# ini/multigrid

Measured on AMD Instinct MI355X. Metric: agent-steps/sec, higher is better.
Workload: dtype u8

## Files before the change

### multigrid_amd/csrc/mgx_fused.h

```cpp
#pragma once
#if !defined(__HIPCC_RTC__)
#include <hip/hip_runtime.h>
#include <limits.h>
#include <stdint.h>
#else
namespace __hip_internal {}
using namespace __hip_internal;
typedef unsigned long uintptr_t;
#ifndef offsetof
#define offsetof(t, m) __builtin_offsetof(t, m)
#endif
#ifndef INT_MAX
#define INT_MAX 2147483647
#endif
#ifndef INT64_MAX
#define INT64_MAX 9223372036854775807LL
#endif
#endif

#include "mgx_rules.h"
#include "mgx_layout_gen.h"

namespace mgx_fused {

// ... 463 lines not shown
        for (int n = 0; n < NH; ++n) {
            uint32_t t, addr;
            asm("v_pk_max_i16 %0, %1, %2" : "=v"(t) : "v"(lc.pk[0]), "v"(r[n].lo));
            asm("v_pk_min_i16 %0, %1, %2" : "=v"(t) : "v"(t), "v"(r[n].hi));
            asm("v_dot2_i32_i16 %0, %1, %2, %3" : "=v"(addr) : "v"(t), "v"(r[n].steps), "v"(r[n].origin));
            MGX_CHECK_LDS_ADDR(4, addr, C8 ? 1 : 2);
            raw[h0 + n] = gather_read<C8>(addr);
        }
        if (h0 + NH < N) __builtin_amdgcn_sched_barrier(0);
    }
#pragma unroll
    for (int p = 0; p < NP; ++p) {
        constexpr int kLast = N - 3 * (NP - 1);
        const int ns = p == NP - 1 ? kLast : 3;
        const int sub16 = ns == 3 ? lc.sub16 : min(lc.sub16, (ns - 1) * (int)sizeof(ViewRec));
        const ViewRec r = *reinterpret_cast<const ViewRec *>(reinterpret_cast<const uint8_t *>(rec + S0 + 3 * p) + sub16);
        uint32_t t, addr;
        asm("v_pk_max_i16 %0, %1, %2" : "=v"(t) : "v"(lc.pk[1]), "v"(r.lo));
        asm("v_pk_min_i16 %0, %1, %2" : "=v"(t) : "v"(t), "v"(r.hi));
        asm("v_dot2_i32_i16 %0, %1, %2, %3" : "=v"(addr) : "v"(t), "v"(r.steps), "v"(r.origin));
        if (lc.act[1]) MGX_CHECK_LDS_ADDR(4, addr, C8 ? 1 : 2);
        rawR[p] = gather_read<C8>(addr);
    }
    [[maybe_unused]] uint32_t dec[C8 ? N : 1], decR[C8 ? NP : 1];
    if constexpr (C8) {
#pragma unroll
        for (int n = 0; n < N; ++n) {
            MGX_CHECK_LDS_ADDR(9, lut_mid + (raw[n] << 2), 4);
            dec[n] = lut_decode(raw[n], lut_mid);
        }
#pragma unroll
        for (int p = 0; p < NP; ++p) {
            if (lc.act[1]) MGX_CHECK_LDS_ADDR(9, lut_mid + (rawR[p] << 2), 4);
            decR[p] = lut_decode(rawR[p], lut_mid);
        }
    }
    uint64_t pend = 0;
#pragma unroll
    for (int n = 0; n < N; ++n) {
        if constexpr (HALF) {
            if ((n & 1) == 0) cell[(S0 + n) >> 1][0] = raw[n] | (raw[n + 1] << 16);
        } else if constexpr (C8) {
            cell[S0 + n][0] = dec[n];
        } else {
            cell[S0 + n][0] = raw[n];
        }
        uint64_t cur;
        if (n == 0) {
            asm volatile("v_cmp_lt_i16_e64 %0, -1, %1\n\ts_nop 1" : "=s"(cur) : "v"(raw[n]));
        } else {
            asm volatile("v_cmp_lt_i16_e64 %0, -1, %3\n\tv_writelane_b32 %1, %4, %6\n\tv_writelane_b32 %2, %5, %6"
                         : "=&s"(cur), "+v"(sbLo[0]), "+v"(sbHi[0])
                         : "v"(raw[n]), "s"((uint32_t)pend), "s"((uint32_t)(pend >> 32)), "n"(S0 + n - 1));
        }
        pend = cur;
    }
    asm volatile("s_nop 1\n\tv_writelane_b32 %0, %2, %4\n\tv_writelane_b32 %1, %3, %4"
                 : "+v"(sbLo[0]), "+v"(sbHi[0]) : "s"((uint32_t)pend), "s"((uint32_t)(pend >> 32)), "n"(S0 + N - 1));
#pragma unroll
    for (int p = 0; p < NP; ++p) {
        constexpr int kLast = N - 3 * (NP - 1);
        const int ns = p == NP - 1 ? kLast : 3;
        if constexpr (C8) cell[pk3_reg<N>(S0, p)][1] = decR[p];
        else cell[pk3_reg<N>(S0, p)][1] = rawR[p];
        uint64_t cur;
        asm volatile("v_cmp_lt_i16_e64 %0, -1, %1" : "=s"(cur) : "v"(rawR[p]));
        constexpr uint32_t kWord = (1u << R) - 1u;
#pragma unroll
        for (int q = 0; q < 3; ++q) {
            if (q < ns) {
                const uint32_t part = (uint32_t)(cur >> (R * q)) & kWord;
                asm volatile("v_writelane_b32 %0, %1, %2" : "+v"(sbLo[1]) : "s"(part), "n"(S0 + 3 * p + q));
            }
        }
    }
    (void)sbHi;
}

#ifndef MGX_GROUP
#define MGX_GROUP 16
#endif
constexpr int kGroup = MGX_GROUP;

template <int V, int NW, int VPW, bool HALF, int G, bool C8 = false, int S0 = 0>
__device__ __forceinline__ void gather_all(const KernelArgs &a, const int wave, int NVc, const ViewRec *rec,
                                           const LaneConst<V, NW> &lc, uint32_t (&cell)[HALF ? VPW / 2 : VPW][NW],
                                           uint32_t (&sbLo)[NW], uint32_t (&sbHi)[NW], const uint32_t lut_mid = 0) {
    if constexpr (S0 < VPW) {
        if (S0 < NVc) {
            if constexpr (kPack3<V>) gather_group_pk3<V, NW, S0, G, VPW, HALF, C8>(a, wave, rec, lc, cell, sbLo, sbHi, lut_mid);
            else gather_group<V, NW, S0, G, VPW, HALF, C8>(a, wave, rec, lc, cell, sbLo, sbHi, lut_mid);
        }
        gather_all<V, NW, VPW, HALF, G, C8, S0 + G>(a, wave, NVc, rec, lc, cell, sbLo, sbHi, lut_mid);
    }
}

template <int V, int MODE, bool HOOKS, bool AR, bool OH = false, bool GEN = false, bool STREAM = false, bool DMA = (MGX_LDS_DMA != 0),
          int GRP = kGroup, int SHAPE = 0, bool C8 = false, bool B3 = false>
__global__ __launch_bounds__(kMaxThreads) void mgx_fused_kernel(const KernelArgs a) {
#include "mgx_fused_body.inc"
}

template <int MODE, bool AR>
__global__ __launch_bounds__(kMaxThreads) __attribute__((amdgpu_waves_per_eu(4)))
void mgx_resident_kernel(const KernelArgs a) {
    constexpr int V = 7, GRP = kGroup, SHAPE = kShapeResident4;
    constexpr bool HOOKS = false, OH = false, GEN = false, STREAM = false, DMA = false, C8 = false, B3 = false;
#include "mgx_fused_body.inc"
}

template <int V, bool OH, bool STREAM, bool DMA, bool C8 = false, bool B3 = false>
__global__ __launch_bounds__(kMaxThreads) __attribute__((amdgpu_waves_per_eu(6)))
void mgx_obs_kernel(const KernelArgs a) {
    constexpr int MODE = 0, GRP = kGroup, SHAPE = 0;
    constexpr bool HOOKS = false, AR = false, GEN = false;
#include "mgx_fused_body.inc"
}

constexpr bool has_small_groups(int V, int MODE, bool OH, bool GEN) {
    return MGX_DEBUG_KNOBS != 0 && MODE == 1 && V <= 9 && !OH && !GEN;
}

inline int match_fixed_shape(const KernelArgs &ka, bool hooks, bool persist = false) {
    if (MGX_NO_FIXED_SHAPES || ka.grp != kGroup) return 0;
    for (int k = 1; k < kNumShapes; ++k) {
        const FixedShape &f = kShapes[k];
        if (f.ns > 0) continue;
        if (persist ? !f.dma : (((ka.flags & 2) != 0) != f.dma || ((ka.flags & 1) != 0) != f.stream)) continue;
        if (ka.sp.view_size == f.V
            && ka.sp.width == f.W && ka.sp.height == f.H && ka.sp.num_agents == f.A && ka.Gw == f.Gw && hooks == f.hooks
            && ka.vpw == shape_slots(f)
            && cell_bytes_of(ka.sp) == f.cb
            && ka.wave_lds == make_carve(f.W, f.H, f.A, f.V, f.Gw, shape_slots(f), persist, f.hooks, false, kGroup, f.cb).total())
            return k;
    }
    return 0;
}

inline int match_resident_shape(const KernelArgs &ka, bool hooks) {
    if (MGX_NO_FIXED_SHAPES || ka.grp != kGroup || ka.ns < 1 || ka.rshape < 1 || ka.rshape >= kNumShapes) return 0;
    const FixedShape &f = kShapes[ka.rshape];
    if (f.ns == ka.ns && ka.sp.view_size == f.V && ka.sp.width == f.W && ka.sp.height == f.H && ka.sp.num_agents == f.A && ka.Gw == f.Gw
        && hooks == f.hooks && ka.vpw == shape_slots(f) && cell_bytes_of(ka.sp) == f.cb && ka.wave_lds == shape_carve(f, true).total())
        return ka.rshape;
    return 0;
}

#if !defined(__HIPCC_RTC__)
struct JitShape { FixedShape f; int vpw, wave_lds; hipFunction_t fn[2]; };
const JitShape *jit_shape_lookup(const KernelArgs &ka, bool hooks);
template <int V, int MODE, bool STREAM, bool C8 = true, bool OH = false>
inline int launch_compact(const KernelArgs &ka, int threads, int lds_bytes, int64_t nwg, hipStream_t stream, int *hip_err, int *occupancy) {
    constexpr bool B3 = !C8;
    if constexpr (MODE > 1 && C8 && !OH && !STREAM) {
        if (ka.grp != kGroup || ka.vpw > 32) return MGX_ERR_INVALID_ARGUMENT;
        if (ka.sp.env_kind != MGX_KIND_EMPTY) return MGX_ERR_UNSUPPORTED;
        const bool ar = ka.pool_grid != nullptr;
        void (*kern)(const KernelArgs) = ar ? mgx_fused_kernel<V, MODE, false, true, false, false, false, false, kGroup, 0, true, false>
                                            : mgx_fused_kernel<V, MODE, false, false, false, false, false, false, kGroup, 0, true, false>;
        if (lds_bytes > 64 * 1024) {
            hipError_t e = hipFuncSetAttribute(reinterpret_cast<const void *>(kern), hipFuncAttributeMaxDynamicSharedMemorySize, lds_bytes);
            if (e != hipSuccess) { *hip_err = (int)e; (void)hipGetLastError(); return MGX_ERR_LAUNCH; }
        }
        if (occupancy) {
            hipError_t e = hipOccupancyMaxActiveBlocksPerMultiprocessor(occupancy, reinterpret_cast<const void *>(kern), threads, (size_t)lds_bytes);
            if (e != hipSuccess) { *hip_err = (int)e; (void)hipGetLastError(); return MGX_ERR_LAUNCH; }
// ... 199 lines not shown
```

### multigrid_amd/csrc/mgx_fused_body.inc

```
    constexpr bool DO_STEP = MODE != 0;
    const int env_kind = HOOKS ? a.sp.env_kind : (int)MGX_KIND_EMPTY;
    constexpr bool PERSIST = MODE == 3;
    constexpr bool ROLL = MODE == 2 || PERSIST;
    constexpr int kOutAux = PERSIST ? 16 : MGX_OUT_AUX;
#define MGX_PUB_STORE_U8(base, idx, n, val)                                                                            \
    do {                                                                                                               \
        if constexpr (PERSIST) __builtin_amdgcn_raw_buffer_store_b8((uint8_t)(val), make_rsrc((base), (n)), (idx), 0, 16); \
        else MGX_STORE_SMALL((base) + (idx), (uint8_t)(val));                                                          \
    } while (0)
    constexpr int V2 = V * V;
    constexpr int NW = (V2 + 63) / 64;
    constexpr int CB = C8 ? 1 : kCellBytes;
    static_assert(!C8 || (!GEN && !DMA && (MODE < 2 ? (!OH || (MODE == 1 && !HOOKS)) : (!OH && !HOOKS))),
                  "compact cells: the plain step / gen_obs kernels, the step with one-hot output, the hook-free rollout / persistent kernels");
    static_assert(SHAPE == 0 || kShapes[SHAPE].cb == CB, "shape table entry of the other cell format");
    static_assert(!B3 || (!C8 && !OH && !GEN && !DMA && MODE < 2 && SHAPE == 0), "byte grids: the plain step / gen_obs kernels only");
    constexpr int CBG = B3 ? 3 : CB;
    constexpr bool RSHAPE = SHAPE != 0 && kShapes[SHAPE].ns > 0;
    constexpr int NS = RSHAPE ? kShapes[SHAPE].ns : 1;
    constexpr int PITCH = RSHAPE ? kShapes[SHAPE].pitch : 0;
    constexpr bool SLICED = RSHAPE && shape_sliced(kShapes[SHAPE]);
    static_assert(!RSHAPE || ((MODE == 2 || MODE == 3) && !OH && !GEN && !STREAM && !DMA && !C8 && !B3 && V <= 7), "resident shapes: rollout / persistent kernels");
    static_assert(NS <= 2, "slices: the (step, slice) sequence below is written for one or two");
    constexpr bool HALF = !DMA && (MODE == 1 || RSHAPE) && !C8;
    constexpr bool PK3 = kPack3<V>;
    constexpr int kG = GRP, kR = SLICED ? kRoundResident : GRP;
    constexpr int kG4 = kR < kG ? kR : kG;
    constexpr int VPW = (DMA && GRP < kGroup) ? GRP : ((V <= 7 && HALF) ? kSlotsSmallView : 32);
    extern __shared__ __align__(16) uint8_t lds[];

    int lane_ = threadIdx.x & 63;
#define lane lane_

    const int wave = __builtin_amdgcn_readfirstlane(threadIdx.x >> 6);
#if MGX_EARLY_ARGS
    if constexpr ((DMA || MGX_EARLY_ARGS > 1) && V <= 7) {
        const int64_t e_batch = a.batch;
        const uint8_t *e_grid = a.grid, *e_agents = a.agents, *e_aux = a.aux, *e_hord = a.hook_order;
        const uint64_t *e_rng = a.rng;
        const int32_t *e_sc = a.step_count;
        const int8_t *e_act = a.actions;
        const unsigned e_bd = blockDim.x;
        const int32_t *e_ep = (AR || GEN) ? a.episode : nullptr;
        const uint8_t *e_trunc = DO_STEP ? a.truncated : nullptr;
        const uint64_t *e_gs = GEN ? a.gen.gen_state : nullptr;
        const int32_t *e_tag = GEN ? a.gen.stage.tag : nullptr;
        asm volatile("" :: "s"(e_batch), "s"(e_grid), "s"(e_agents), "s"(e_rng), "s"(e_sc), "s"(e_act), "s"(e_hord), "s"(e_aux),
                     "s"(e_bd), "s"(e_ep), "s"(e_trunc), "s"(e_gs), "s"(e_tag));
    }
#endif
    constexpr bool FIXED = SHAPE != 0;
    constexpr bool PREFIX = FIXED ? (kShapes[SHAPE].A > 4) : (V > 7 && MODE == 1);
    constexpr bool BIGCOPY = FIXED ? (kShapes[SHAPE].W * kShapes[SHAPE].H * CB >= 4096) : (V > 7 && MODE == 1);
    const int W = FIXED ? kShapes[SHAPE].W : a.sp.width, H = FIXED ? kShapes[SHAPE].H : a.sp.height,
              A = FIXED ? kShapes[SHAPE].A : a.sp.num_agents;
    const int Gw_ = FIXED ? kShapes[SHAPE].Gw : a.Gw;
    const int vpw_ = FIXED ? shape_slots(kShapes[SHAPE]) : a.vpw;
    const int inv_A_ = FIXED ? (65536 + kShapes[SHAPE].A - 1) / (FIXED ? kShapes[SHAPE].A : 1) : a.inv_A;
    const int HWB = H * W * CB;
    const int HWG = H * W * CBG;
#define MGX_LATE_GEN(f) kernarg_at<decltype(MgxLayoutGen::f)>(offsetof(KernelArgs, gen) + offsetof(MgxLayoutGen, f))
#define MGX_LATE_STAGE(f) kernarg_at<decltype(MgxGenStage::f)>(offsetof(KernelArgs, gen) + offsetof(MgxLayoutGen, stage) + offsetof(MgxGenStage, f))
    if constexpr (GEN && MODE == 1) {
        if ((int64_t)blockIdx.x >= a.gen_first_wg) {
            const int64_t gw = ((int64_t)blockIdx.x - a.gen_first_wg) * (blockDim.x >> 6) + wave;
            const int64_t b = gw * 64 + lane;
            int32_t *const tag = MGX_LATE_STAGE(tag);
            const int32_t phase1 = MGX_LATE_STAGE(phase) + 1;
            const bool serial = MGX_LATE_STAGE(external) == 2;
            int32_t req = b >= a.batch ? 0 : serial ? tag[b * 4 + 3]
                                                    : __hip_atomic_load(tag + b * 4 + 3, __ATOMIC_ACQUIRE, __HIP_MEMORY_SCOPE_AGENT);
            if (req != 0 && req != phase1 && tag[b * 4 + 1] != a.episode[b]) { tag[b * 4 + 3] = 0; req = 0; }
            const bool go = req != 0 && req != phase1;
            const uint64_t gom = __builtin_amdgcn_ballot_w64(go);
#if MGX_SPANS
            const int64_t wid_g = a.gen_first_wg * (blockDim.x >> 6) + gw;
            const unsigned long long t_g0 = __builtin_amdgcn_s_memrealtime();
            if (gom == 0 && lane == 0 && a.span_base + wid_g < kSpanCap) {
                g_span[2 * (a.span_base + wid_g)] = t_g0;
                g_span[2 * (a.span_base + wid_g) + 1] = __builtin_amdgcn_s_memrealtime() & 0x0fffffffffffffffull;
            }
#endif
            if (gom == 0) return;
            MGX_RARE_PATH_PRIO();
            MgxLayoutGen gen;
            gen.kind = MGX_LATE_GEN(kind); gen.room_size = MGX_LATE_GEN(room_size);
            gen.start_x = MGX_LATE_GEN(start_x); gen.start_y = MGX_LATE_GEN(start_y); gen.start_dir = MGX_LATE_GEN(start_dir);
            gen.max_hallway_keys = MGX_LATE_GEN(max_hallway_keys); gen.max_keys_per_room = MGX_LATE_GEN(max_keys_per_room);
            gen.blank = MGX_LATE_GEN(blank); gen.gen_state = MGX_LATE_GEN(gen_state);
            uint8_t *const st_grid = reinterpret_cast<uint8_t *>(MGX_LATE_STAGE(grid));
            mgx_gen::copy_blank(gen, st_grid, gw * 64, HWB, gom, lane);
            __builtin_amdgcn_fence(__ATOMIC_RELEASE, "wavefront");
            __builtin_amdgcn_s_waitcnt(0x0F70);
            wave_sync();
            if (go) {
                const int32_t ep_s = tag[b * 4 + 1], sc_s = tag[b * 4 + 2];
                uint64_t *const words = MGX_LATE_STAGE(words) + b * 12;
                const uint64_t *gs = gen.gen_state + b * 6, *rg = a.rng + b * 4;
                mgx_gen::NpGen lay, npr;
                for (int k = 0; k < 4; ++k) lay.s[k] = gs[k];
                lay.buf = gs[4]; npr.buf = gs[5];
                uint64_t s0 = words[10], s1 = words[11];
                const uint64_t i0 = rg[2], i1 = rg[3];
                const uint64_t jA[4] = {kJump.w[A][0], kJump.w[A][1], kJump.w[A][2], kJump.w[A][3]};
                if (A > 1 && a.sp.max_steps > sc_s) pcg64_advance(s0, s1, i0, i1, jA, (uint32_t)(a.sp.max_steps - sc_s));
                npr.s[0] = s0; npr.s[1] = s1; npr.s[2] = i0; npr.s[3] = i1;
                uint8_t *apos = lds + wave * a.wave_lds + lane * (2 * A);
                const uint4 naux = mgx_gen::generate_episode(gen, W, H, A, lay, npr, apos, st_grid + b * HWB,
// ... 781 lines not shown
        if (ovl >= 0) {
            MGX_CHECK_LDS_PTR(3, mytile + ovl, CB);
            store_cell_raw(CB, mytile + ovl, agent_cell_raw(CB, cur_row));
        }
    } else {
        const int off = (lane < NVc) ? overlay_offset(cf, rows + env_of_lane * A, agent_of_lane) : -1;
        wave_sync();
        if (off >= 0) store_cell_raw(CB, tile + env_of_lane * TSB + off, agent_cell_raw(CB, cur_row));
    }
    wave_sync();

    MGX_MARK("P1d");
    const uint32_t tile_addr = (uint32_t)(wave * wave_lds_ + cv.tile(sl_s) + tile_skew);
    uint32_t my_carry = 0;
    uint8_t *const p_dir = MGX_LATE(dir);
    uint8_t *const p_agents = DO_STEP ? MGX_LATE(agents) : nullptr;
    double *const p_reward = DO_STEP ? MGX_LATE(reward) : nullptr;
    uint8_t *const p_term = DO_STEP ? MGX_LATE(terminated) : nullptr;
    if (lane < NVc) {
        const int e = env_of_lane;
        const uint64_t row = cur_row;
        const ViewGeom g = view_geom<V>(W, H, row_x(row), row_y(row), row_dir(row), CB, PITCH);
        const ViewClamp vc = view_clamp<V>(g, W, H, row_x(row), row_y(row));
        ViewRec r;
        r.origin = vc.valid ? (int32_t)tile_addr + e * TSB + g.origin : (int32_t)wall_addr;
        r.steps = vc.valid ? vc.steps : 0u; r.lo = vc.valid ? vc.lo : 0u; r.hi = vc.valid ? vc.hi : 0u;
        my_carry = row_carry(row) & kCellShown;
        rec[lane] = r;
        if (DO_STEP) {
            const u32x2 rowv = {(uint32_t)row, (uint32_t)(row >> 32)};
            if (!ROLL) __builtin_amdgcn_raw_buffer_store_b64(rowv, make_rsrc(p_agents + v0 * 8, NVc * 8), lane * 8, 0,MGX_OUT_AUX);
            const uint64_t rbits = __builtin_bit_cast(uint64_t, my_rew);
            const u32x2 rewv = {(uint32_t)rbits, (uint32_t)(rbits >> 32)};
            __builtin_amdgcn_raw_buffer_store_b64(rewv, make_rsrc(p_reward + tv0, NVc * 8), lane * 8, 0, kOutAux);
            const bool forced = env_kind == MGX_KIND_LOCKEDHALLWAY && reinterpret_cast<const uint8_t *>(auxl + e)[15];
            __builtin_amdgcn_raw_buffer_store_b8((uint8_t)(row_term(row) | forced),
                                                 make_rsrc(p_term + tv0, NVc), lane, 0, kOutAux);
        }
        if (p_dir) __builtin_amdgcn_raw_buffer_store_b8((uint8_t)row_dir(row), make_rsrc(p_dir + tv0, NVc), lane, 0, kOutAux);
    } else if (lane < ((NVc + kG - 1) & ~(kG - 1))) {
        ViewRec r;
        r.origin = (int32_t)wall_addr; r.steps = 0; r.lo = 0; r.hi = 0;
        rec[lane] = r;
    }
    wave_sync();

    if constexpr (GEN && MODE == 1) {
        const uint64_t alive_now = __builtin_amdgcn_ballot_w64(lane < NVc && !row_term(cur_row));
        if (lane < Gc) {
            const uint64_t amask = (A >= 64) ? ~0ull : ((1ull << A) - 1ull);
            done_now = (((alive_now >> mad24(lane, A, 0)) & amask) == 0) | ((int32_t)in_scnt + 1 >= cf.max_steps);
            uint8_t *wr = MGX_LATE(was_reset);
            if (wr) wr[e0 + lane] = (uint8_t)done_now;
        }
        done_mask = __builtin_amdgcn_ballot_w64(done_now);
        if (stage_tag && cand_K > 0) {
            const bool dn = done_now;
            if (done_mask != 0) {
                cand_r = cand_draw(cand_npr);
                const int r = cand_r;
                const int32_t tr = (int32_t)(r == 0 ? in_tags.x : r == 1 ? in_tags.y : r == 2 ? in_tags.z : in_tags.w);
                cand_mask = __builtin_amdgcn_ballot_w64(dn && tr == (int32_t)in_ep);
                if (cand_mask != 0 && (HWB & 3) == 0 && HWB <= 1024) {
                    pre_e = __builtin_ctzll(cand_mask);
                    const int64_t s = (e0 + pre_e) * cand_K + __builtin_amdgcn_readlane(r, pre_e);
                    const uint32_t *sg = reinterpret_cast<const uint32_t *>(reinterpret_cast<const uint8_t *>(MGX_LATE_STAGE(grid)) + s * HWB);
                    const int nd = HWB / 4;
#pragma unroll
                    for (int k = 0; k < 4; ++k) pre_grid[k] = (lane + 64 * k < nd) ? sg[lane + 64 * k] : 0u;
                    pre_row = lane < A ? (reinterpret_cast<const uint64_t *>(MGX_LATE_STAGE(agents)) + s * A)[lane] : 0ull;
                    pre_word = lane < 5 ? (MGX_LATE_STAGE(words) + s * 6)[lane] : 0ull;
                    if (HOOKS) pre_aux = reinterpret_cast<const uint4 *>(MGX_LATE_STAGE(aux))[s];
                }
            }
        }
    }

    MGX_MARK("P2");
    const LaneConst<V, NW> lc = ROLL ? lc_roll : lane_consts();
    uint32_t cell[HALF ? VPW / 2 : VPW][NW];
    uint32_t sbLo[NW], sbHi[NW];
#pragma unroll
    for (int k = 0; k < NW; ++k) { sbLo[k] = 0; sbHi[k] = 0; }
    if (!MGX_DBG(4)) gather_all<V, NW, VPW, HALF, kG, C8>(a, wave, NVc, rec, lc, cell, sbLo, sbHi,
                                                          (uint32_t)(wave * wave_lds_ + cv.lut() + 512));
    if (ROLL) {
        wave_sync();
        if (ovl_off >= 0) store_cell_raw(CB, tile + env_of_lane * TSB + ovl_off, ovl_saved);
    }

    MGX_MARK("P3");
    const bool masked = !a.sp.see_through_walls;
    uint32_t visLo[NW], visHi[NW];
#pragma unroll
    for (int k = 0; k < NW; ++k) { visLo[k] = 0xffffffffu; visHi[k] = 0xffffffffu; }
    if (masked && !MGX_DBG(8)) {
        uint64_t sb[NW], vis[NW];
#pragma unroll
        for (int k = 0; k < NW; ++k) sb[k] = ((uint64_t)sbHi[k] << 32) | sbLo[k];
        constexpr int kOwn = (V - 1) * V + V / 2;
        sb[kOwn >> 6] = (sb[kOwn >> 6] & ~(1ull << (kOwn & 63)))
                      | ((uint64_t)see_behind(my_carry) << (kOwn & 63));
        vis_mask<V, NW>(sb, vis);
#pragma unroll
        for (int k = 0; k < NW; ++k) { visLo[k] = (uint32_t)vis[k]; visHi[k] = (uint32_t)(vis[k] >> 32); }
    }

    MGX_MARK("P4");
    auto slot_cell = [&](const int s, const int it) -> uint32_t {
        if constexpr (HALF) return (s & 1) ? cell[s >> 1][it] >> 16 : cell[s >> 1][it];
        else return cell[s][it];
    };
    auto to_obs = [](const uint32_t c) -> uint32_t { if constexpr (C8) return c; else return cell_unpack(c); };
    if constexpr (OH) {
        constexpr int D = 21;
        constexpr uint32_t kInvD = 0xFFFFFFFFu / D + 1u;
        const int64_t h0 = tv0 * (int64_t)(V2 * D), h1 = h0 + (int64_t)NVc * V2 * D;
        const int oh_skew = (int)(h0 & 15);
        uint32_t *masks = reinterpret_cast<uint32_t *>(L + cv.out()) + 1;
        auto one_hot_mask = [](uint32_t c) -> uint32_t { return one_hot_mask21(c); };
        constexpr uint32_t kUnseenMask = 1u | (1u << 11) | (1u << 17);
        auto cell_mask = [&](const bool seen, const uint32_t x) -> uint32_t {
            if constexpr (C8) return seen ? x : kUnseenMask;
            else return one_hot_mask(to_obs(seen ? x : CELL_UNSEEN));
        };
        if (lane == 0) masks[-1] = 0;
#pragma unroll
        for (int r0 = 0; r0 < VPW; r0 += kR) {
            if (r0 < NVc) {
#pragma unroll
                for (int it = 0; it < NW; ++it) {
                    if (lc.act[it]) {
                        uint32_t *d0 = masks + (lc.q3[it] / 3);
                        if constexpr (PK3) {
                            if (it == 1) {
                                constexpr int R = V2 - 64, NP = pack3_passes(kG), kLast = kG - 3 * (NP - 1);
#pragma unroll
                                for (int g0 = 0; g0 < kR; g0 += kG) {
                                    if (r0 + g0 < NVc) {
#pragma unroll
                                        for (int p = 0; p < NP; ++p) {
                                            const int ns = p == NP - 1 ? kLast : 3, sl = g0 + 3 * p, s = r0 + sl;
                                            uint64_t m = (uint64_t)(uint32_t)__builtin_amdgcn_readlane(visLo[1], s);
                                            if (ns > 1) m |= (uint64_t)(uint32_t)__builtin_amdgcn_readlane(visLo[1], s + 1) << R;
                                            if (ns > 2) m |= (uint64_t)(uint32_t)__builtin_amdgcn_readlane(visLo[1], s + 2) << (2 * R);
                                            const uint32_t x = C8 ? cell[pk3_reg<kG>(r0 + g0, p)][1] : (cell[pk3_reg<kG>(r0 + g0, p)][1] & 0xffffu);
                                            if (ns == 3 || lane < ns * R) {
                                                MGX_CHECK_LDS_PTR(7, d0 + sl * V2, 4);
                                                d0[sl * V2] = cell_mask(__builtin_amdgcn_inverse_ballot_w64(m), x);
                                            }
                                        }
                                    }
                                }
                                continue;
                            }
                        }
#pragma unroll
                        for (int g0 = 0; g0 < kR; g0 += kG) {
                            if (r0 + g0 < NVc) {
#pragma unroll
                                for (int sl = g0; sl < g0 + kG; ++sl) {
                                    const int s = r0 + sl;
                                    const uint64_t m = (V2 - 64 * it > 32 ? (uint64_t)(uint32_t)__builtin_amdgcn_readlane(visHi[it], s) << 32 : 0ull)
                                                     | (uint64_t)(uint32_t)__builtin_amdgcn_readlane(visLo[it], s);
                                    MGX_CHECK_LDS_PTR(7, d0 + sl * V2, 4);
                                    d0[sl * V2] = cell_mask(__builtin_amdgcn_inverse_ballot_w64(m), slot_cell(s, it));
                                }
                            }
                        }
                    }
                }
                wave_sync();
                if (lane >= r0 && lane < r0 + kR && lane < NVc)
                    masks[(lane - r0) * V2 + (V / 2) * V + (V - 1)] = one_hot_mask(my_carry);
                wave_sync();
                MGX_MARK("P5");
                const int64_t ro0 = h0 + (int64_t)r0 * (V2 * D);
                const int rbytes = (int)min((int64_t)kR * V2 * D, h1 - ro0);
                const int rlen = oh_skew + rbytes;
                uint8_t *gdst = MGX_LATE(obs) + (ro0 - oh_skew);
                const __amdgpu_buffer_rsrc_t orsrc = make_rsrc(gdst, rlen);
                for (int rel = lane16; rel < rlen; rel += 1024) {
                    const uint32_t xs = (uint32_t)(rel - oh_skew + D);
                    const uint32_t cq = __umulhi(xs, kInvD);
                    const uint32_t k0 = xs - cq * D;
                    MGX_CHECK_LDS_PTR(8, masks + (int)cq - 1, 8);
                    const uint32_t bits = (masks[(int)cq - 1] >> k0) | (masks[(int)cq] << (D - k0));
                    u32x4 v;
                    v.x = (((bits >> 0) & 0xfu) * 0x00204081u) & 0x01010101u;
                    v.y = (((bits >> 4) & 0xfu) * 0x00204081u) & 0x01010101u;
                    v.z = (((bits >> 8) & 0xfu) * 0x00204081u) & 0x01010101u;
                    v.w = (((bits >> 12) & 0xfu) * 0x00204081u) & 0x01010101u;
                    if ((rel + 16 <= rlen) & (rel >= oh_skew)) {
                        __builtin_amdgcn_raw_buffer_store_b128(v, orsrc, rel, 0, PERSIST ? 16 : MGX_OH_AUX);
                    } else {
                        const int lo_b = max(rel, oh_skew), hi_b = min(rel + 16, rlen);
#pragma clang loop vectorize(disable) unroll(disable)
                        for (int B = lo_b; B < hi_b; ++B) {
                            const int q = (B - rel) >> 2;
                            const uint32_t w = q == 0 ? v.x : (q == 1 ? v.y : (q == 2 ? v.z : v.w));
                            __builtin_amdgcn_raw_buffer_store_b8((uint8_t)(w >> (8 * ((B - rel) & 3))), orsrc, B, 0, PERSIST ? 16 : 0);
                        }
                    }
                }
                wave_sync();
                MGX_MARK("P5end");
            }
        }
    } else {
    [[maybe_unused]] const int64_t o0 = tv0 * (int64_t)(V2 * 3), o1 = o0 + (int64_t)NVc * V2 * 3;
    if constexpr (obs_dword_staging(V, ROLL)) {
    static_assert(NW == 1 && !PK3 && !PERSIST && kR % 4 == 0, "dword staging: views of one lane pass, rounds of whole dwords");
    uint32_t *const stg = reinterpret_cast<uint32_t *>(L + cv.out()) + 4;
    const int s_w = (int)(o0 & 3);
    const __amdgpu_buffer_rsrc_t orsrc = make_rsrc(MGX_LATE(obs) + (o0 - s_w), s_w + NVc * V2 * 3);
    constexpr int kUnits = kR * V2 / 4 + 1;
    constexpr int kPasses = (kUnits + 63) / 64;
    uint32_t *const d0 = stg + lc.q3[0] / 3;
    auto p5_whole = [&](const int r0) {
        constexpr int kWhole = kR * V2 / 4, kWP = (kWhole + 63) / 64;
        u32x4 d[kWP];
#pragma unroll
        for (int k = 0; k < kWP; ++k) {
            const int u = 64 * (k + 1) <= kWhole ? lane + 64 * k : min(lane + 64 * k, kWhole - 1);
            MGX_CHECK_LDS_PTR(6, stg + 4 * u, 16);
            d[k] = *reinterpret_cast<const u32x4 *>(stg + 4 * u);
        }
#pragma unroll
        for (int k = 0; k < kWP; ++k) {
            uint32_t w[3];
            obs_unit(0u, d[k].x, d[k].y, d[k].z, d[k].w, 0, w);
            if (64 * (k + 1) <= kWhole || lane + 64 * k < kWhole)
                __builtin_amdgcn_raw_buffer_store_b96(u32x3{w[0], w[1], w[2]}, orsrc, 12 * (lane + 64 * k), r0 * V2 * 3,
                                                      STREAM ? MGX_OBS_AUX : MGX_OBS_AUX_CACHED);
        }
    };
    auto p5_round = [&](const int r0, const int s) {
        const int roff = r0 * V2 * 3;
        const int ulen = s + (int)min(kR * V2 * 3, (NVc - r0) * V2 * 3);
#pragma unroll
        for (int k = 0; k < kPasses; ++k) {
            const int u = lane + 64 * k, ub = 12 * u;
            if (ub < ulen) {
                MGX_CHECK_LDS_PTR(6, stg + 4 * u - 1, 20);
                const u32x4 d = *reinterpret_cast<const u32x4 *>(stg + 4 * u);
                const uint32_t dm1 = s ? stg[4 * u - 1] : 0u;
                uint32_t w[3];
                obs_unit(dm1, d.x, d.y, d.z, d.w, s, w);
                if (ub >= s && ub + 12 <= ulen) {
                    __builtin_amdgcn_raw_buffer_store_b96(u32x3{w[0], w[1], w[2]}, orsrc, ub, roff, STREAM ? MGX_OBS_AUX : MGX_OBS_AUX_CACHED);
                } else {
                    const int lo_b = max(s - ub, 0), hi_b = min(ulen - ub, 12);
#pragma clang loop vectorize(disable) unroll(disable)
                    for (int B = lo_b; B < hi_b; ++B) {
                        const uint32_t x = B < 4 ? w[0] : (B < 8 ? w[1] : w[2]);
                        __builtin_amdgcn_raw_buffer_store_b8((uint8_t)(x >> (8 * (B & 3))), orsrc, ub + B, roff, 0);
                    }
                }
            }
        }
    };
#pragma unroll
    for (int r0 = 0; r0 < VPW; r0 += kR) {
        if (r0 < NVc) {
            if (!MGX_DBG(16)) {
                if (lc.act[0]) {
#pragma unroll
                    for (int g0 = 0; g0 < kR; g0 += kG4) {
                        if (r0 + g0 < NVc) {
#pragma unroll
                            for (int sl = g0; sl < g0 + kG4; ++sl) {
                                const int s = r0 + sl;
                                const uint64_t m = (V2 > 32 ? (uint64_t)(uint32_t)__builtin_amdgcn_readlane(visHi[0], s) << 32 : 0ull)
                                                 | (uint64_t)(uint32_t)__builtin_amdgcn_readlane(visLo[0], s);
                                const uint32_t x = HALF ? cell[s >> 1][0] : cell[s][0];
                                const uint32_t c = C8 ? x : perm_b32((x >> 12) & 0x00030003u, x & 0x070f070fu, obs_stage_sel(HALF && (s & 1)));
                                MGX_CHECK_LDS_PTR(5, d0 + sl * V2, 4);
                                d0[sl * V2] = __builtin_amdgcn_inverse_ballot_w64(m) ? c : 0u;
                            }
                        }
                    }
                }
                wave_sync();
                if (lane >= r0 && lane < r0 + kR && lane < NVc) {
                    MGX_CHECK_LDS_PTR(5, stg + (lane - r0) * V2 + (V / 2) * V + (V - 1), 4);
                    stg[(lane - r0) * V2 + (V / 2) * V + (V - 1)] = my_carry;
                }
            }
            wave_sync();
            MGX_MARK("P5");
            if (!MGX_DBG(32)) {
                if (s_w == 0 && r0 + kR <= NVc) p5_whole(r0);
                else p5_round(r0, s_w);
            }
            wave_sync();
            MGX_MARK("P5end");
        }
    }
    } else {
    const int out_skew0 = (int)(o0 & 15);
    uint8_t *out_raw = L + cv.out();
    constexpr int kRoundBytes = kR * V2 * 3;
#pragma unroll
    for (int r0 = 0; r0 < VPW; r0 += kR) {
        const int out_skew = (kRoundBytes & 15) ? ((out_skew0 + ((r0 * V2 * 3) & 15)) & 15) : out_skew0;
        uint8_t *const outb = out_raw + out_skew;
        if (r0 < NVc) {
            if (!MGX_DBG(16)) {
#pragma unroll
                for (int it = 0; it < NW; ++it) {
                    if (lc.act[it]) {
                        uint8_t *d0 = outb + lc.q3[it];
                        const uint32_t par0 = (uint32_t)(out_skew + lc.q3[it]) & 1u;
                        uint8_t *const d16[2] = {d0 + par0, d0 + (par0 ^ 1u)};
                        uint8_t *const d8[2] = {d0 + 2u * (par0 ^ 1u), d0 + 2u * par0};
                        const uint32_t sel[2] = {C8 ? (par0 ? 0x0c000201u : 0x0c020100u) : (par0 ? 0x0c000401u : 0x0c040100u),
                                                 C8 ? (par0 ? 0x0c020100u : 0x0c000201u)
                                                    : (HALF ? (par0 ? 0x0c060302u : 0x0c020603u) : (par0 ? 0x0c040100u : 0x0c000401u))};
                        if constexpr (PK3) {
                            if (it == 1) {
                                constexpr int R = V2 - 64, NP = pack3_passes(kG), kLast = kG - 3 * (NP - 1);
                                const uint32_t selR[2] = {C8 ? sel[0] : (par0 ? 0x0c000401u : 0x0c040100u),
                                                          C8 ? sel[1] : (par0 ? 0x0c040100u : 0x0c000401u)};
#pragma unroll
                                for (int g0 = 0; g0 < kR; g0 += kG) {
                                    if (r0 + g0 < NVc) {
#pragma unroll
                                        for (int p = 0; p < NP; ++p) {
                                            const int ns = p == NP - 1 ? kLast : 3, sl = g0 + 3 * p, s = r0 + sl;
                                            uint64_t m = (uint64_t)(uint32_t)__builtin_amdgcn_readlane(visLo[1], s);
                                            if (ns > 1) m |= (uint64_t)(uint32_t)__builtin_amdgcn_readlane(visLo[1], s + 1) << R;
                                            if (ns > 2) m |= (uint64_t)(uint32_t)__builtin_amdgcn_readlane(visLo[1], s + 2) << (2 * R);
                                            const uint32_t x = cell[pk3_reg<kG>(r0 + g0, p)][1];
                                            const uint32_t tc = C8 ? x : (x & 0x070fu), st = C8 ? x : ((x >> 12) & 0x0003u);
                                            const uint32_t pr = __builtin_amdgcn_perm(st, tc, selR[sl & 1]);
                                            const uint32_t c = __builtin_amdgcn_inverse_ballot_w64(m) ? pr : 0u;
                                            if (ns == 3 || lane < ns * R) {
                                                MGX_CHECK_LDS_PTR(5, d0 + sl * (V2 * 3), 3);
                                                *reinterpret_cast<uint16_t *>(d16[sl & 1] + sl * (V2 * 3)) = (uint16_t)c;
                                                d8[sl & 1][sl * (V2 * 3)] = (uint8_t)(c >> 16);
                                            }
                                        }
                                    }
                                }
                                continue;
                            }
                        }
#pragma unroll
// ... 285 lines not shown
```

### multigrid_amd/csrc/mgx_rules.h

```cpp
#pragma once
#if !defined(__HIPCC_RTC__)
#include <stdint.h>
#endif

#include "../../include/mgx.h"

#if defined(__HIPCC__)
#define MGX_HD __host__ __device__ __forceinline__
#else
#define MGX_HD inline
#endif

namespace mgx {

enum : int { T_UNSEEN = 0, T_EMPTY = 1, T_WALL = 2, T_FLOOR = 3, T_DOOR = 4, T_KEY = 5, T_BALL = 6, T_BOX = 7,
             T_GOAL = 8, T_LAVA = 9, T_AGENT = 10 };
enum : int { S_OPEN = 0, S_CLOSED = 1, S_LOCKED = 2 };
enum : int { ACT_LEFT = 0, ACT_RIGHT = 1, ACT_FORWARD = 2, ACT_PICKUP = 3, ACT_DROP = 4, ACT_TOGGLE = 5, ACT_DONE = 6 };
enum : int { AG_COLOR = 0, AG_DIR = 1, AG_X = 2, AG_Y = 3, AG_TERM = 4, AG_CARRY = 5 };

constexpr uint32_t kCellShown = 0x0003ffffu;
constexpr uint32_t CELL_EMPTY = 1u;
constexpr uint32_t CELL_WALL = 2u | (5u << 8);
constexpr uint32_t CELL_UNSEEN = 0u;
// ... 498 lines not shown
MGX_HD void overlay_agents(const StepCfg &cf, uint8_t *tile, const uint64_t *rows) {
    if (cf.A <= 1) return;
    for (int a = 0; a < cf.A; ++a) {
        const uint64_t r = rows[a];
        if (row_term(r)) continue;
        const int x = row_x(r), y = row_y(r);
        if (x >= cf.W || y >= cf.H) continue;
        store_cell_raw(cf.cb, tile + (y * cf.P + x) * cf.cb, agent_cell_raw(cf.cb, r));
    }
}

MGX_HD int overlay_offset(const StepCfg &cf, const uint64_t *rows, int ai) {
    if (cf.A <= 1) return -1;
    const uint64_t r = rows[ai];
    const uint32_t pos = ((uint32_t)r >> 16) & 0xffffu;
    bool shadowed = false;
#pragma unroll 4
    for (int j = 0; j < cf.A; ++j) {
        const uint64_t o = rows[j];
        shadowed |= (j > ai) & !row_term(o) & ((((uint32_t)o >> 16) & 0xffffu) == pos);
    }
    const int x = row_x(r), y = row_y(r);
    if (row_term(r) | shadowed | (x >= cf.W) | (y >= cf.H)) return -1;
    return (y * cf.P + x) * cf.cb;
}

MGX_HD uint32_t fastmod_u32(uint32_t a, uint64_t M, uint32_t d) {
    const uint64_t low = M * a;
    const uint64_t hi_part = (low >> 32) * d, lo_part = (low & 0xffffffffull) * d;
    return (uint32_t)((hi_part + (lo_part >> 32)) >> 32);
}
MGX_HD int pool_index(int64_t first_env, int64_t b, int32_t ep, int32_t K, uint64_t M) {
    if (K == 1) return 0;
    const uint64_t g = (uint64_t)(first_env + b);
    if (K <= (1 << 19) && (g >> 32) == 0 && ep >= 0) {
        const uint32_t k = (uint32_t)K;
        const uint32_t x = fastmod_u32((uint32_t)g, M, k) + fastmod_u32((uint32_t)ep, M, k) * (7919u % k);
        return (int)fastmod_u32(x, M, k);
    }
    return (int)((uint64_t)(first_env + b + (int64_t)ep * 7919) % (uint64_t)K);
}

struct ViewGeom { int origin, stepF, stepL, fmax, imin, imax; };

template <int V>
MGX_HD ViewGeom view_geom(int W, int H, int x, int y, int d, int cb = kCellBytes, int pitch = 0) {
    const int dx = dir_dx(d), dy = dir_dy(d), h = V / 2;
    const int P = pitch ? pitch : W;
    ViewGeom g;
    g.origin = (y * P + x) * cb;
    g.stepF = (dy * P + dx) * cb;
    g.stepL = (dx * P - dy) * cb;
    const bool d0 = d == 0, d1 = d == 1, d2 = d == 2;
    g.fmax = d0 ? W - 1 - x : (d1 ? H - 1 - y : (d2 ? x : y));
    const int lmin = d0 ? -y : (d1 ? x - (W - 1) : (d2 ? y - (H - 1) : -x));
    const int lmax = d0 ? H - 1 - y : (d1 ? x : (d2 ? y : W - 1 - x));
    g.imin = lmin + h < 0 ? 0 : lmin + h;
    g.imax = lmax + h > V - 1 ? V - 1 : lmax + h;
    return g;
}

struct ViewClamp { uint32_t steps, lo, hi; bool valid; };

template <int V>
MGX_HD ViewClamp view_clamp(const ViewGeom &g, int W, int H, int x, int y) {
    constexpr int h = V / 2;
    ViewClamp c;
    const int fhi = g.fmax > V - 1 ? V - 1 : g.fmax;
    c.steps = ((uint32_t)g.stepF & 0xffffu) | ((uint32_t)g.stepL << 16);
    c.lo = (uint32_t)(g.imin - h) << 16;
    c.hi = ((uint32_t)fhi & 0xffffu) | ((uint32_t)(g.imax - h) << 16);
    c.valid = (x < W) & (y < H) & (g.fmax >= 0) & (g.imax >= g.imin);
    return c;
}

MGX_HD int clamped_offset(int origin, const ViewClamp &c, int fw, int la) {
    auto lo16 = [](uint32_t v) { return (int)(int16_t)(v & 0xffffu); };
    auto hi16 = [](uint32_t v) { return (int)(int16_t)(v >> 16); };
    int f = fw > lo16(c.lo) ? fw : lo16(c.lo), l = la > hi16(c.lo) ? la : hi16(c.lo);
    f = f < lo16(c.hi) ? f : lo16(c.hi); l = l < hi16(c.hi) ? l : hi16(c.hi);
    return origin + f * lo16(c.steps) + l * hi16(c.steps);
}

template <int V, int NW>
MGX_HD void inbounds_mask(const ViewGeom &g, uint64_t (&m)[NW]) {
    const bool any = g.imax >= g.imin;
    const uint32_t cols = any ? (((2u << g.imax) - 1u) & ~((1u << g.imin) - 1u)) : 0u;
    const int jmin = (V - 1 - g.fmax) < 0 ? 0 : (V - 1 - g.fmax);
    if constexpr (NW == 1) {
        uint64_t r = cols;
        r |= r << V;
        r |= r << (2 * V);
        if (V > 4) r |= r << (4 * V);
        constexpr uint64_t kAll = (V * V >= 64) ? ~0ull : ((1ull << ((V * V) & 63)) - 1ull);
        m[0] = (jmin >= V) ? 0ull : (r & kAll & (~0ull << (jmin * V)));
    } else {
        for (int k = 0; k < NW; ++k) m[k] = 0;
#pragma unroll
        for (int j = 0; j < V; ++j)
            if (j >= jmin) or_bits<V, NW>(m, j * V, cols);
    }
}

}
```

Measured before the change: 14.25 billion.

## Gather agent views by rows with eight-lane line mapping and compute visibility per view

Adds a row-per-lane mapping for small views in one-step kernels: each group of eight lanes gathers one view, with each lane reading one row of up to V cells. A per-row opaque byte goes to LDS, then one lane per view computes the visibility mask with a row-wise propagation. The staging loop writes cells through per-row visibility bytes instead of per-cell readlane/inverse-ballot. This is meant to cut per-slot readlane and ballot overhead and the cross-lane see-behind packing, at the cost of extra LDS round trips and wave syncs.

```diff
diff --git a/multigrid_amd/csrc/mgx_fused.h b/multigrid_amd/csrc/mgx_fused.h
--- a/multigrid_amd/csrc/mgx_fused.h
+++ b/multigrid_amd/csrc/mgx_fused.h
@@ -569,6 +569,52 @@
 #endif
 constexpr int kGroup = MGX_GROUP;
 
+__host__ __device__ __attribute__((always_inline)) constexpr bool view_line_lanes(int V, bool roll, bool one_hot, bool c8, int grp) {
+    return obs_dword_staging(V, roll) && V <= kLineLanes && !one_hot && !c8 && grp == kGroup && kGroup % kLineLanes == 0;
+}
+
+template <int V, int I>
+__device__ __forceinline__ void line_reads(const KernelArgs &a, const int wave, const int base, const int la_lo, const int la_hi,
+                                           const int stepL, uint32_t (&raw)[V]) {
+    if constexpr (I < V) {
+        const uint32_t addr = (uint32_t)line_cell_offset<I - V / 2>(base, la_lo, la_hi, stepL);
+        MGX_CHECK_LDS_ADDR(10, addr, 2);
+        raw[I] = gather_read<false>(addr);
+        line_reads<V, I + 1>(a, wave, base, la_lo, la_hi, stepL, raw);
+    }
+}
+
+template <int V, int VPW, int S0>
+__device__ __forceinline__ void gather_lines(const KernelArgs &a, const int wave, const int lane, const int NVc, const ViewRec *rec,
+                                             uint8_t *bytes, uint32_t (&cellp)[VPW / kLineLanes][(V + 1) / 2]) {
+    if constexpr (S0 < VPW) {
+        if (S0 < NVc) {
+            constexpr int P0 = S0 / kLineLanes, PN = kGroup / kLineLanes;
+            const int j = lane & (kLineLanes - 1);
+            ViewRec r[PN];
+#pragma unroll
+            for (int q = 0; q < PN; ++q) {
+                MGX_CHECK_LDS_ADDR(11, (uint32_t)(uintptr_t)(lds_u32_ptr)(const void *)(rec + (P0 + q) * kLineLanes + (lane >> 3)), sizeof(ViewRec));
+                r[q] = rec[(P0 + q) * kLineLanes + (lane >> 3)];
+            }
+            uint32_t raw[PN][V];
+#pragma unroll
+            for (int q = 0; q < PN; ++q)
+                line_reads<V, 0>(a, wave, line_base(r[q].origin, r[q].steps, r[q].lo, r[q].hi, V - 1 - j), clamp_hi16(r[q].lo),
+                                 clamp_hi16(r[q].hi), clamp_hi16(r[q].steps), raw[q]);
+#pragma unroll
+            for (int q = 0; q < PN; ++q) {
+#pragma unroll
+                for (int k = 0; k < (V + 1) / 2; ++k)
+                    cellp[P0 + q][k] = 2 * k + 1 < V ? (raw[q][2 * k] | (raw[q][2 * k + 1] << 16)) : raw[q][2 * k];
+                MGX_CHECK_LDS_ADDR(12, (uint32_t)(uintptr_t)(lds_u32_ptr)(const void *)(bytes + (P0 + q) * 64 + lane), 1);
+                bytes[(P0 + q) * 64 + lane] = (uint8_t)line_opaque_byte<V>(cellp[P0 + q]);
+            }
+        }
+        gather_lines<V, VPW, S0 + kGroup>(a, wave, lane, NVc, rec, bytes, cellp);
+    }
+}
+
 template <int V, int NW, int VPW, bool HALF, int G, bool C8 = false, int S0 = 0>
 __device__ __forceinline__ void gather_all(const KernelArgs &a, const int wave, int NVc, const ViewRec *rec,
                                            const LaneConst<V, NW> &lc, uint32_t (&cell)[HALF ? VPW / 2 : VPW][NW],
diff --git a/multigrid_amd/csrc/mgx_fused_body.inc b/multigrid_amd/csrc/mgx_fused_body.inc
--- a/multigrid_amd/csrc/mgx_fused_body.inc
+++ b/multigrid_amd/csrc/mgx_fused_body.inc
@@ -24,6 +24,7 @@
     static_assert(NS <= 2, "slices: the (step, slice) sequence below is written for one or two");
     constexpr bool HALF = !DMA && (MODE == 1 || RSHAPE) && !C8;
     constexpr bool PK3 = kPack3<V>;
+    constexpr bool LINES = view_line_lanes(V, ROLL, OH, C8, GRP);
     constexpr int kG = GRP, kR = SLICED ? kRoundResident : GRP;
     constexpr int kG4 = kR < kG ? kR : kG;
     constexpr int VPW = (DMA && GRP < kGroup) ? GRP : ((V <= 7 && HALF) ? kSlotsSmallView : 32);
@@ -971,6 +972,12 @@
     uint32_t sbLo[NW], sbHi[NW];
 #pragma unroll
     for (int k = 0; k < NW; ++k) { sbLo[k] = 0; sbHi[k] = 0; }
+    [[maybe_unused]] uint32_t cellp[LINES ? VPW / kLineLanes : 1][(V + 1) / 2];
+    [[maybe_unused]] uint8_t *const line_bytes = L + cv.rows();
+    if constexpr (LINES) {
+        static_assert(!ROLL && !SLICED && NW == 1 && VPW % kGroup == 0, "line map: one-step kernels, views of one lane pass");
+        if (!MGX_DBG(4)) gather_lines<V, VPW, 0>(a, wave, lane, NVc, rec, line_bytes, cellp);
+    } else
     if (!MGX_DBG(4)) gather_all<V, NW, VPW, HALF, kG, C8>(a, wave, NVc, rec, lc, cell, sbLo, sbHi,
                                                           (uint32_t)(wave * wave_lds_ + cv.lut() + 512));
     if (ROLL) {
@@ -983,6 +990,22 @@
     uint32_t visLo[NW], visHi[NW];
 #pragma unroll
     for (int k = 0; k < NW; ++k) { visLo[k] = 0xffffffffu; visHi[k] = 0xffffffffu; }
+    if constexpr (LINES) {
+        wave_sync();
+        if (lane < NVc) {
+            u32x2 *const w = reinterpret_cast<u32x2 *>(line_bytes) + lane;
+            MGX_CHECK_LDS_PTR(13, w, 8);
+            uint64_t vis = ~0ull;
+            if (masked && !MGX_DBG(8)) {
+                const u32x2 sbw = *w;
+                const uint64_t sb = (~(((uint64_t)sbw.y << 32) | sbw.x) & ~(1ull << kLineOwnBit<V>))
+                                  | ((uint64_t)see_behind(my_carry) << kLineOwnBit<V>);
+                vis = vis_mask_lines<V>(sb);
+            }
+            *w = u32x2{(uint32_t)vis, (uint32_t)(vis >> 32)};
+        }
+        wave_sync();
+    } else
     if (masked && !MGX_DBG(8)) {
         uint64_t sb[NW], vis[NW];
 #pragma unroll
@@ -1149,10 +1172,42 @@
             }
         }
     };
+    [[maybe_unused]] uint32_t line_vis[LINES ? VPW / kLineLanes : 1];
+    if constexpr (LINES) {
+#pragma unroll
+        for (int p = 0; p < VPW / kLineLanes; ++p) {
+            line_vis[p] = 0;
+            if (p * kLineLanes / kR * kR < NVc) {
+                MGX_CHECK_LDS_PTR(14, line_bytes + p * 64 + lane, 1);
+                line_vis[p] = line_bytes[p * 64 + lane];
+            }
+        }
+    }
 #pragma unroll
     for (int r0 = 0; r0 < VPW; r0 += kR) {
         if (r0 < NVc) {
             if (!MGX_DBG(16)) {
+                if constexpr (LINES) {
+                    constexpr int PR = kR / kLineLanes;
+                    const int lj = lane & (kLineLanes - 1);
+                    if (lj < V) {
+                        uint32_t *const dl = stg + (lane >> 3) * V2 + lj;
+#pragma unroll
+                        for (int q = 0; q < PR; ++q) {
+                            const uint32_t vb = line_vis[r0 / kLineLanes + q];
+#pragma unroll
+                            for (int k = 0; k < (V + 1) / 2; ++k) {
+                                const uint32_t x = cellp[r0 / kLineLanes + q][k];
+                                const uint32_t tc = x & 0x070f070fu, st = (x >> 12) & 0x00030003u;
+#pragma unroll
+                                for (int i = 2 * k; i < 2 * k + 2 && i < V; ++i) {
+                                    MGX_CHECK_LDS_PTR(5, dl + q * kLineLanes * V2 + i * V, 4);
+                                    dl[q * kLineLanes * V2 + i * V] = line_stage_cell(tc, st, i, vb);
+                                }
+                            }
+                        }
+                    }
+                } else
                 if (lc.act[0]) {
 #pragma unroll
                     for (int g0 = 0; g0 < kR; g0 += kG4) {
diff --git a/multigrid_amd/csrc/mgx_rules.h b/multigrid_amd/csrc/mgx_rules.h
--- a/multigrid_amd/csrc/mgx_rules.h
+++ b/multigrid_amd/csrc/mgx_rules.h
@@ -604,6 +604,74 @@
     return origin + f * lo16(c.steps) + l * hi16(c.steps);
 }
 
+constexpr int kLineLanes = 8;
+
+MGX_HD int clamp_hi16(uint32_t v) { return (int32_t)v >> 16; }
+
+MGX_HD int line_base(int origin, uint32_t steps, uint32_t lo, uint32_t hi, int fw) {
+#if defined(__HIP_DEVICE_COMPILE__)
+    uint32_t t;
+    int r;
+    asm("v_pk_max_i16 %0, %1, %2" : "=v"(t) : "v"((uint32_t)fw & 0xffffu), "v"(lo));
+    asm("v_pk_min_i16 %0, %1, %2" : "=v"(t) : "v"(t), "v"(hi));
+    asm("v_dot2_i32_i16 %0, %1, %2, %3" : "=v"(r) : "v"(t & 0xffffu), "v"(steps), "v"(origin));
+    return r;
+#else
+    const int l = (int)(int16_t)(lo & 0xffffu), h = (int)(int16_t)(hi & 0xffffu);
+    int f = fw > l ? fw : l;
+    f = f < h ? f : h;
+    return origin + f * (int)(int16_t)(steps & 0xffffu);
+#endif
+}
+
+template <int LA>
+MGX_HD int line_cell_offset(int base, int la_lo, int la_hi, int stepL) {
+#if defined(__HIP_DEVICE_COMPILE__)
+    int l, r;
+    asm("v_med3_i32 %0, %1, %2, %3" : "=v"(l) : "n"(LA), "v"(la_lo), "v"(la_hi));
+    asm("v_mad_i32_i24 %0, %1, %2, %3" : "=v"(r) : "v"(l), "v"(stepL), "v"(base));
+    return r;
+#else
+    const int mn = la_lo < la_hi ? la_lo : la_hi, mx = la_lo < la_hi ? la_hi : la_lo;
+    const int l = LA < mn ? mn : (LA > mx ? mx : LA);
+    return base + l * stepL;
+#endif
+}
+
+template <int V>
+MGX_HD uint32_t line_opaque_byte(const uint32_t (&pr)[(V + 1) / 2]) {
+    uint32_t acc = 0;
+#pragma unroll
+    for (int k = 0; k < (V + 1) / 2; ++k) acc |= ((pr[k] & 0x80008000u) >> 15) << (2 * k);
+    return (acc | (acc >> 15)) & 0xffu;
+}
+
+template <int V>
+MGX_HD uint64_t vis_mask_lines(uint64_t sb) {
+    static_assert(V <= kLineLanes && V * kLineLanes <= 64, "line map: views of up to 8 rows of up to 8 cells");
+    constexpr uint32_t F = (1u << V) - 1u;
+    uint64_t vis = 0;
+    uint32_t init = 1u << (V / 2);
+    init |= brev32(init);
+#pragma unroll
+    for (int j = V - 1; j >= 0; --j) {
+        const uint32_t s0 = (uint32_t)(sb >> (kLineLanes * j)) & F;
+        const uint32_t s = s0 | brev32(s0);
+        uint32_t u = ((s + (init & s)) ^ s) | init;
+        u |= brev32(u);
+        vis |= (uint64_t)(u & F) << (kLineLanes * j);
+        const uint32_t p = u & s;
+        init = p | (p << 1) | (p >> 1);
+    }
+    return vis;
+}
+template <int V> constexpr int kLineOwnBit = (V - 1) * kLineLanes + V / 2;
+
+MGX_HD uint32_t line_stage_cell(uint32_t tc, uint32_t st, int i, uint32_t vis_byte) {
+    const uint32_t c = perm_b32(st, tc, obs_stage_sel((i & 1) != 0));
+    return c & (uint32_t)((int32_t)(vis_byte << (31 - i)) >> 31);
+}
+
 template <int V, int NW>
 MGX_HD void inbounds_mask(const ViewGeom &g, uint64_t (&m)[NW]) {
     const bool any = g.imax >= g.imin;
```

Result: faster. 16.00 billion (median of 6 runs) (+12.3%).
